# atonderski/future-object-detection

Measured on AMD Instinct MI355X. Metric: frame-sequences/sec fwd+bwd, T=6 900x1600, higher is better.
Workload: dtype bf16; 1 GPU; spatiotemporal ConditionalDETR (ResNet-50, 6 enc + 6 dec layers, 128 queries), T=6 frames 900x1600, batch 2/GPU, num_images K=5 (5 past frames live), random-init weights; step = forward (incl. Hungarian set loss, post-proc, AP bookkeeping) + backward + clip + AdamW; global_batch=2, frames=6, num_images=5, parallelism=dp1

## Files before the change

future-object-detection_amd/csrc/api.cpp:

```cpp
#include <stdarg.h>
#include <stdio.h>
#include <string.h>

#include "../../include/fod.h"

static thread_local char g_err[512] = "";

void fod_set_error(const char* fmt, ...) {
  va_list ap;
  va_start(ap, fmt);
  vsnprintf(g_err, sizeof(g_err), fmt, ap);
  va_end(ap);
}

extern "C" size_t fod_last_error(char* buf, size_t cap) {
  const size_t n = strlen(g_err);
  if (buf && cap) {
    const size_t c = n < cap - 1 ? n : cap - 1;
    memcpy(buf, g_err, c);
    buf[c] = 0;
  }
  return n;
}

extern "C" int fod_abi_version(void) { return FOD_ABI_VERSION; }

extern "C" size_t fod_workspace_bytes(int kind) {
  switch (kind) {
    case FOD_WS_NT_SPLIT: return (size_t)FOD_NT_SPLIT_WS_FLOATS * sizeof(float);
    case FOD_WS_NT_SPLIT_TICKETS: return (size_t)FOD_NT_SPLIT_TICKETS * sizeof(unsigned);
    case FOD_WS_TN_PARTIALS: return FOD_TN_WS_BYTES;
    case FOD_WS_ATTN_SPLIT_PER_TILE: return (size_t)FOD_ATTN_SPLIT_WS_FLOATS_PER_TILE * sizeof(float);
    default: return 0;
  }
}
```

future-object-detection_amd/csrc/gemm_tn_big.hip:

```cpp
#include <stdlib.h>

#include <type_traits>

#include "common.h"
#include "gemm_tn.h"
#include "lds_dma.h"

namespace {

using namespace fodtn;

constexpr int MS = 64;
constexpr int tn_stages(int bi, int bj) { return bi + bj == 512 ? 2 : 3; }
constexpr int tn_stage_bytes(int bi, int bj) { return MS * (bi + bj) * 2; }

template <int PITCH>
FOD_DEVINL Frag<__bf16> tr_frag(const unsigned char* tile, int a0, int ks) {
  typedef __attribute__((address_space(3))) short4_t* lds_s4;
  const short4_t lo = __builtin_amdgcn_ds_read_tr16_b64_v4i16((lds_s4)(tile + a0 + ks * 16 * PITCH));
  const short4_t hi = __builtin_amdgcn_ds_read_tr16_b64_v4i16((lds_s4)(tile + a0 + ks * 16 * PITCH + 4 * PITCH));
  typedef __attribute__((ext_vector_type(8))) short short8_t;
  const short8_t v = __builtin_shufflevector(lo, hi, 0, 1, 2, 3, 4, 5, 6, 7);
  Frag<__bf16> f;
  __builtin_memcpy(&f, &v, 16);
  return f;
}

template <int MODE, int BI, int BJ>
__global__ __launch_bounds__(512) void tn_big_kernel(const TnParams p) {
  static_assert((BI + BJ == 384 && (BI == 128 || BI == 256)) || (BI == 256 && BJ == 256),
                "tile shapes: 128 x 256, 256 x 128 or 256 x 256");
  constexpr int NSTAGE = tn_stages(BI, BJ), STAGE_BYTES = tn_stage_bytes(BI, BJ);
  constexpr int PG = BI * 2, PX = BJ * 2;
  constexpr int G_BYTES = MS * PG;
  constexpr int G_DMA = BI / 64, X_DMA = BJ / 64;
  constexpr int N_DMA = G_DMA + X_DMA;
  constexpr int WTJ = BI * BJ / 8 / 64;
  constexpr int NB = WTJ / 32;
  constexpr int WJ = BJ / WTJ;
  constexpr unsigned OOB = 0xFFFFFFF0u;
  extern __shared__ __attribute__((aligned(16))) unsigned char smem[];

  const int tid = threadIdx.x;
  const int lane = tid & 63;
  const int wave = __builtin_amdgcn_readfirstlane(tid >> 6);
  const int wi = wave / WJ, wj = wave % WJ;
  BLK_STAMP(0);
  const int ntile = p.ti * p.tj;
  const int per = (ntile * p.nsplit + 7) >> 3;
  const int item = p.xcd_order ? (int)(blockIdx.x & 7) * per + (int)(blockIdx.x >> 3) : (int)blockIdx.x;
  if (p.xcd_order && (int)(blockIdx.x >> 3) >= per) return;
  const int split = item / ntile;
  const int tile = item - split * ntile;
  const int bx = tile % p.tj, by = tile / p.tj;
  if (split >= p.nsplit) return;
  const int j0 = bx * BJ, i0 = by * BI;
  const int mb = split * p.m_per_split;
  const int mend = min(p.M, mb + p.m_per_split);
  const int nst = (mend - mb + MS - 1) / MS;

  const v4i rsG = make_rsrc(p.G, p.g_bytes), rsX = make_rsrc(p.X, p.x_bytes);
  const unsigned lds0 = (unsigned)(uintptr_t)(lds_ptr)smem;

  unsigned g_off[G_DMA];
  int g_m[G_DMA];
#pragma unroll
  for (int i = 0; i < G_DMA; ++i) {
    constexpr int CPR = PG / 16, RPP = 1024 / PG;
    const int row = (wave + 8 * i) * RPP + lane / CPR;
    const int sc = (lane % CPR) ^ ((row & 3) << 2);
    const int col = i0 + sc * 8;
    g_m[i] = col < p.N1 ? mb + row : (1 << 30);
    g_off[i] = (unsigned)(((long)(mb + row) * p.ldg + col) * 2);
  }
  const unsigned g_step = (unsigned)((long)MS * p.ldg * 2);

  unsigned x_off[X_DMA];
  int x_m[X_DMA];
// ... 209 lines not shown
      for (int a = 0; a < 2; ++a)
#pragma unroll
        for (int r = 0; r < 16; ++r)
          mine[(wi * 64 + a * 32 + acc_row(r, lane)) * BJ + wj * WTJ + b * 32 + (lane & 31)] = acc[a][b][r] * rs[a][r];
  } else {
#pragma unroll
    for (int b = 0; b < NB; ++b) {
      const int j = j0 + wj * WTJ + b * 32 + (lane & 31);
#pragma unroll
      for (int a = 0; a < 2; ++a)
#pragma unroll
        for (int r = 0; r < 16; ++r) {
          const int i = i0 + wi * 64 + a * 32 + acc_row(r, lane);
          if (i < p.N1 && j < p.K2) atomicAdd(p.dW + (long)i * p.ldw + j, acc[a][b][r] * rs[a][r]);
        }
    }
  }
#ifdef FOD_STAMPS
  asm volatile("s_waitcnt vmcnt(0)" ::: "memory");
  BLK_STAMP(3);
#endif
}

template <int BI, int BJ>
__global__ __launch_bounds__(256) void tn_reduce_kernel(const TnParams p) {
  __shared__ f32x4 red[3][64];
  const int c4 = p.K2 >> 2;
  const int chunks = (c4 + 63) >> 6;
  const int i = blockIdx.x / chunks;
  const int j4 = (blockIdx.x - i * chunks) * 64 + (threadIdx.x & 63);
  const int q = threadIdx.x >> 6;
  const bool in = j4 < c4;
  const int j = min(j4, c4 - 1) * 4;
  const int ntile = p.ti * p.tj;
  const int tile = (i / BI) * p.tj + j / BJ;
  const float* src = p.ws + (long)tile * (BI * BJ) + (i % BI) * BJ + j % BJ;
  const long stride = (long)ntile * (BI * BJ);
  f32x4 acc = {0.f, 0.f, 0.f, 0.f};
  int s = q;
  for (; s + 12 < p.nsplit; s += 16) {
    const f32x4 v0 = *reinterpret_cast<const f32x4*>(src + (s + 0) * stride);
    const f32x4 v1 = *reinterpret_cast<const f32x4*>(src + (s + 4) * stride);
    const f32x4 v2 = *reinterpret_cast<const f32x4*>(src + (s + 8) * stride);
    const f32x4 v3 = *reinterpret_cast<const f32x4*>(src + (s + 12) * stride);
    acc += v0;
    acc += v1;
    acc += v2;
    acc += v3;
  }
  for (; s < p.nsplit; s += 4) acc += *reinterpret_cast<const f32x4*>(src + s * stride);
  if (q > 0) red[q - 1][threadIdx.x & 63] = acc;
  __syncthreads();
  if (q > 0 || !in) return;
  acc += red[0][threadIdx.x];
  acc += red[1][threadIdx.x];
  acc += red[2][threadIdx.x];
  float* dst = p.dW + (long)i * p.ldw + j;
  if (p.accumulate) acc += *reinterpret_cast<const f32x4*>(dst);
  *reinterpret_cast<f32x4*>(dst) = acc;
}

template <int MODE, int BI, int BJ>
int launch_shape(const TnParams& p, hipStream_t stream) {
  static LdsLimitOnce lds_once;
  const size_t lds = (size_t)tn_stages(BI, BJ) * tn_stage_bytes(BI, BJ);
  if (int rc = fod_lds_limit_once(lds_once, reinterpret_cast<const void*>(&tn_big_kernel<MODE, BI, BJ>), lds, "gemm_tn_big")) return rc;
  const int ntile = p.ti * p.tj;
  const dim3 grid(p.xcd_order ? 8 * ceil_div((long)ntile * p.nsplit, 8) : ntile * p.nsplit);
  TnParams q = p;
  q.ws = nullptr;
  const char* env_ws = getenv("FOD_TN_WS");
  const size_t need = (size_t)ntile * p.nsplit * BI * BJ * sizeof(float);
  const bool aligned = ((uintptr_t)p.dW % 16) == 0 && p.ldw % 4 == 0;
  if (p.nsplit > 1 && p.ws_caller && need <= p.ws_caller_bytes && aligned && ((uintptr_t)p.ws_caller % 16) == 0 &&
      !(env_ws && env_ws[0] == '0'))
    q.ws = p.ws_caller;
  hipLaunchKernelGGL((tn_big_kernel<MODE, BI, BJ>), grid, dim3(512), lds, stream, q);
  FOD_LAUNCH_CHECK();
  if (q.ws) {
    hipLaunchKernelGGL((tn_reduce_kernel<BI, BJ>), dim3(p.N1 * ceil_div(p.K2 / 4, 64)), dim3(256), 0, stream, q);
    FOD_LAUNCH_CHECK();
  }
// ... 10 lines not shown
  const int sq = env_sq ? atoi(env_sq) : 0;
  const bool square = (sq == 2 && p.N1 >= 256 && p.K2 >= 256) ||
                      (sq == 1 && p.N1 % 256 == 0 && p.K2 % 256 == 0 && p.M >= 256 * 64);
  for (int shape = square ? 2 : 0; shape < (square ? 3 : 2); ++shape) {
    const int bi = shape == 0 ? 128 : 256, bj = shape == 2 ? 256 : 384 - bi;
    const int ti = ceil_div(p.N1, bi), tj = ceil_div(p.K2, bj);
    const int ntile = ti * tj;
    int s = 256 / ntile;
    const int max_s = p.M / 256;
    if (s > max_s) s = max_s;
    if (s < 1) s = 1;
    const int mps = ceil_div(ceil_div(p.M, s), MS) * MS;
    const int ns = ceil_div(p.M, mps);
    const int rounds = ceil_div((long)ntile * ns, 256);
    const double cost = rounds * (mps / MS * 0.55 + 17.0);
    if (cost < best_cost) {
      best_cost = cost;
      best = Plan{bi, bj, ti, tj, ns, mps};
    }
  }
  return best;
}

}

namespace fodtn {

bool big_applies(int mode, int dtype, const TnParams& p) {
  const char* env = getenv("FOD_TN_BIG");
  if (env && env[0] == '0') return false;
  if (dtype != FOD_BF16 || p.g_seg_cols) return false;
  if (p.N1 % 8 != 0 || p.K2 % 8 != 0 || p.ldg % 8 != 0) return false;
  if (mode == MODE_DENSE && p.ldx % 8 != 0) return false;
  if (mode == MODE_CONV && p.Cs % 8 != 0) return false;
  if (mode == MODE_CONV && (long)p.Hs * p.Ws * p.Cs * 2 >= (1L << 31)) return false;
  if (env && env[0] == '2') return p.M >= 1;
  const char* env_min = getenv("FOD_TN_BIG_MIN");
  return p.M >= 8192 && p.N1 >= 128 && p.K2 >= 128 && (double)p.M * p.N1 * p.K2 >= (env_min ? atof(env_min) : 2.0e9);
}

int launch_big_mode(int mode, const TnParams& p, hipStream_t stream) {
  TnParams q = p;
  const Plan pl = plan(p);
  q.ti = pl.ti; q.tj = pl.tj; q.nsplit = pl.nsplit; q.m_per_split = pl.m_per_split;
  const char* env_x = getenv("FOD_TN_XCD");
  q.xcd_order = (env_x && env_x[0] == '0') ? 0 : 1;
// ... 20 lines not shown
```

future-object-detection_amd/future_od/native/backbone.py:

```python
import os

import torch
import torch.nn as nn
from torch.autograd import Function

from . import functional as Fn
from . import ops

RESNET_SPECS = {"resnet18": ("basic", (2, 2, 2, 2), 1),
                "resnet34": ("basic", (3, 4, 6, 3), 1),
                "resnet50": ("bottleneck", (3, 4, 6, 3), 4)}
STAGE_WIDTH = (64, 128, 256, 512)


class FrozenBatchNorm2d(nn.Module):

    def __init__(self, n):
        super().__init__()
        self.register_buffer("weight", torch.ones(n))
        self.register_buffer("bias", torch.zeros(n))
        self.register_buffer("running_mean", torch.zeros(n))
        self.register_buffer("running_var", torch.ones(n))
        self.eps = 1e-5

# ... 80 lines not shown
            return ()
        c = getattr(self, "_pixel_norm", None)
        if c is None or c[0].device != video.device:
            c = (torch.tensor(self.PIXEL_MEAN, dtype=torch.float32, device=video.device),
                 torch.tensor(self.PIXEL_STD, dtype=torch.float32, device=video.device))
            object.__setattr__(self, "_pixel_norm", c)
        return c


FUSED_STEM_POOL = os.environ.get("FOD_FUSED_STEM_POOL", "1") != "0"

FRONT_FRAMES = int(os.environ.get("FOD_FRONT_FRAMES", "0")) or (1 << 30)


def _conv_fwd(x, cw, bn, dtype, relu, residual=None, cin_pad=None, out=None):
    scale, shift = bn.scale_shift()
    w = Fn.prep_conv(cw.weight, dtype, scale, False, cin_pad=cin_pad)
    geom = ops.conv_geom(x.shape, cw.weight.shape[0], cw.k, cw.stride, cw.pad)
    return ops.conv2d_fwd(x, w, geom, shift=shift, residual=residual, relu=relu, work_cin=cw.weight.shape[1],
                          out=out), geom


FUSED_BOTTLENECK = os.environ.get("FOD_FUSED_BOTTLENECK", "2")


def _fusable(blk, x, dtype, force=False):
    if (FUSED_BOTTLENECK == "0" and not force) or dtype != torch.bfloat16 or blk.kind == "basic":
        return False
    if FUSED_BOTTLENECK == "1" and not force and blk.downsample is None:
        return False
    main, ds = blk.convs()
    c1, c2, c3 = main[0][0], main[1][0], main[2][0]
    cin = x.shape[-1]
    if c1.weight.shape[0] != 64 or c3.weight.shape[0] != 256 or c2.stride != 1 or c1.stride != 1:
        return False
    if ds is None:
        return cin == 256
    return cin == 64 and ds[0].k == 1 and ds[0].stride == 1


def _fused_bottleneck(blk, x, dtype, out=None):
    main, ds = blk.convs()
    ws, bs = [], []
    for cw, bn in main + ([ds] if ds is not None else []):
        scale, shift = bn.scale_shift()
        ws.append(Fn.prep_conv(cw.weight, dtype, scale, False))
# ... 112 lines not shown
            x, acts, geoms, ds_geom = block_fwd(blk, x, pads=dom)
            if blk.convs()[0][0][0].weight.requires_grad:
                tape.append((blk, acts, geoms, ds_geom, dom))
        if dom is not None:
            x = _parity_merge(x, *dom)
        geom_p = ops.conv_geom(x.shape, proj.weight.shape[0], 1, 1, 0)
        wp = Fn.prep_conv(proj.weight, dtype, None, False)
        feat = ops.conv2d_fwd(x, wp, geom_p, shift=proj.bias.detach())
        ctx.body, ctx.proj, ctx.dtype = body, proj, dtype
        ctx.tape, ctx.x_last, ctx.geom_p = tape, x, geom_p
        ctx.train_weights = train_weights
        return feat

    @staticmethod
    def backward(ctx, dfeat):
        dtype, proj = ctx.dtype, ctx.proj
        dev = dfeat.device
        g = dfeat.contiguous()
        grads = {}
        sync = Fn.GRAD_SYNC
        if sync is not None:
            sync.flush(Fn.ARENA)

        def wgrad(gy, xin, cw, geom, scale):
            co, ci, kh, kw = cw.weight.shape
            dw = Fn.zeros_f32((co, kh, kw, ci), dev)
            ops.conv2d_wgrad_acc(gy, xin, dw, geom, row_scale=scale, zeroed=True)
            grads[id(cw.weight)] = dw.view(co, ci, 1, 1) if kh == 1 and kw == 1 else dw.permute(0, 3, 1, 2)

        if proj.weight.requires_grad:
            wgrad(g, ctx.x_last, proj, ctx.geom_p, None)
            db = Fn.zeros_f32((proj.weight.shape[0],), dev)
            ops.colsum_acc(g.view(-1, g.shape[-1]), db)
            grads[id(proj.bias)] = db
        tape = ctx.tape
        if tape:
            g = ops.conv2d_dgrad(g, Fn.prep_conv(proj.weight, dtype, None, True), ctx.geom_p, relu_mask=ctx.x_last)
        gdom = None
        for bi in range(len(tape) - 1, -1, -1):
            blk, acts, geoms, ds_geom, dom = tape[bi]
            if dom is not None and gdom is None:
                g, gdom = _parity_split(g), dom
            elif dom is None and gdom is not None:
                g, gdom = _parity_merge(g, *gdom), None
            main, ds = blk.convs()
            need_dx = bi > 0
            g_out = g
            gcur = g_out
            for j in range(len(main) - 1, -1, -1):
                cw, bn = main[j]
                scale, _ = bn.scale_shift()
                wgrad(gcur, acts[j], cw, geoms[j], scale)
                if j > 0:
                    gcur = ops.conv2d_dgrad(gcur, Fn.prep_conv(cw.weight, dtype, scale, True), geoms[j],
                                            relu_mask=acts[j])
            if ds is not None:
                wgrad(g_out, acts[0], ds[0], ds_geom, ds[1].scale_shift()[0])
            if need_dx:
                cw, bn = main[0]
                sc = bn.scale_shift()[0]
                w1t = Fn.prep_conv(cw.weight, dtype, sc, True)
                if ds is not None and ds[0].k == 1 and ds[0].stride == 2 and cw.stride == 1 and cw.k == 1:
                    g = ops.conv2d_dgrad(gcur, w1t, geoms[0], relu_mask=acts[0])
                    scd = ds[1].scale_shift()[0]
                    ops.conv2d_dgrad(g_out, Fn.prep_conv(ds[0].weight, dtype, scd, True), ds_geom, residual=g,
                                     relu_mask=acts[0], out=g)
                else:
                    if ds is not None:
                        scd = ds[1].scale_shift()[0]
                        d_idt = ops.conv2d_dgrad(g_out, Fn.prep_conv(ds[0].weight, dtype, scd, True), ds_geom)
                    else:
                        d_idt = g_out
                    g = ops.conv2d_dgrad(gcur, w1t, geoms[0], residual=d_idt, relu_mask=acts[0])
            if sync is not None:
                sync.maybe_flush(Fn.ARENA)
        ctx.tape = None
        out = [None, None, None, None]
        for w in ctx.train_weights:
            out.append(grads.get(id(w)))
        return tuple(out)


def backbone_trainable(body, proj):
    ws = []
    for _stage, blk in body.blocks():
        main, ds = blk.convs()
        for cw, _bn in main + ([ds] if ds is not None else []):
            if cw.weight.requires_grad:
                ws.append(cw.weight)
    ws += [proj.weight, proj.bias]
    return ws


def run_backbone(video, body, proj, dtype):
    feat = BackboneFn.apply(video, body, proj, dtype, *backbone_trainable(body, proj))
    if Fn.BACKBONE_CUT is not None and feat.requires_grad:
# ... 3 lines not shown
```

future-object-detection_amd/future_od/native/lib.py:

```python
import ctypes as C
import os

_HERE = os.path.dirname(os.path.abspath(__file__))
LIB_PATH = os.path.normpath(os.path.join(_HERE, "..", "..", "lib", "libfod_hip.so"))
ABI_VERSION = 4

F32, BF16 = 0, 1
EW_ADD, EW_MUL, EW_RELU_MASK, EW_SCALE, EW_ADD3, EW_RELU, EW_COPY_B = range(7)


class FodError(RuntimeError):
    pass


class Epilogue(C.Structure):
    _fields_ = [("scale", C.c_void_p), ("shift", C.c_void_p), ("residual", C.c_void_p),
                ("ld_residual", C.c_long), ("residual_row_mod", C.c_int), ("relu_mask", C.c_void_p),
                ("ld_mask", C.c_long), ("relu", C.c_int), ("out_f32", C.c_int),
                ("split_ws", C.c_void_p), ("split_tickets", C.c_void_p)]


class ConvGeom(C.Structure):
    _fields_ = [("Nimg", C.c_int), ("H", C.c_int), ("W", C.c_int), ("Cin", C.c_int),
                ("Ho", C.c_int), ("Wo", C.c_int), ("Cout", C.c_int),
                ("kh", C.c_int), ("kw", C.c_int), ("stride", C.c_int), ("pad", C.c_int)]


class AttnShape(C.Structure):
    _fields_ = [("B", C.c_int), ("H", C.c_int), ("Tq", C.c_int), ("S", C.c_int),
                ("q_batch_stride", C.c_long), ("q_token_stride", C.c_long),
                ("k_batch_stride", C.c_long), ("k_token_stride", C.c_long),
                ("v_batch_stride", C.c_long), ("v_token_stride", C.c_long),
                ("o_batch_stride", C.c_long), ("o_token_stride", C.c_long),
                ("scale", C.c_float),
                ("k2_batch_stride", C.c_long), ("k2_token_stride", C.c_long),
                ("dk2_batch_stride", C.c_long), ("dk2_token_stride", C.c_long),
                ("drop_p", C.c_float), ("drop_seed", C.c_ulonglong), ("drop_seed_dev", C.c_void_p),
                ("split_ws", C.c_void_p), ("split_tickets", C.c_void_p), ("dq_scale", C.c_float)]


class PermuteJob(C.Structure):
    _fields_ = [("src", C.c_void_p), ("dst", C.c_void_p), ("scale", C.c_void_p),
                ("src_dtype", C.c_int), ("dst_dtype", C.c_int),
                ("d0", C.c_int), ("d1", C.c_int), ("d2", C.c_int),
                ("valid1", C.c_int), ("valid2", C.c_int), ("scale_axis", C.c_int),
                ("s0", C.c_long), ("s1", C.c_long), ("s2", C.c_long),
                ("t0", C.c_long), ("t1", C.c_long)]

# ... 7 lines not shown


_i, _l, _f, _p = C.c_int, C.c_long, C.c_float, C.c_void_p
_EP, _CG, _AS = _p, _p, _p

SIGNATURES = {
    "fod_gemm_nt": [_i, _p, _l, _i, _p, _l, _p, _l, _i, _i, _i, _EP, _p],
    "fod_gemm_tn_acc": [_i, _p, _l, _p, _l, _p, _l, _i, _i, _i, _p, _p, _i, _p, C.c_size_t, _p],
    "fod_gemm_nt_grouped": [_i, _p, _l, _i, _l, _p, _l, _p, _l, _i, _l, _i, _i, _i, _EP, _i, _l, _p],
    "fod_gemm_nt_batched": [_i, _i, _p, _l, _l, _p, _l, _l, _p, _l, _l, _i, _i, _i, _EP, _l, _l, _l, _p],
    "fod_gemm_tn_grouped": [_i, _p, _l, _i, _l, _p, _l, _p, _l, _i, _i, _i, _p, _i, _p],
    "fod_gemm_tn_multi": [_p, _p, _p, _i, _p],
    "fod_gemm_tn_multi_long": [_p, _p, _p, _i, _p],
    "fod_tn_plan_long": [_i, _i, _p, _p],
    "fod_colsum_acc": [_i, _p, _l, _i, _i, _i, _p, _p],
    "fod_conv2d_fwd": [_i, _p, _p, _p, _CG, _EP, _p],
    "fod_conv2d_dgrad": [_i, _p, _p, _p, _CG, _EP, _p],
    "fod_conv_stem_fwd": [_i, _p, _p, _p, _i, _i, _i, _i, _i, _i, _EP, _p],
    "fod_stem_pool_fwd": [_i, _p, _p, _p, _p, _i, _i, _i, _i, _i, _i, _p],
    "fod_linear_add_norm_fwd": [_i, _p, _l, _p, _p, _p, _p, _p, _p, _p, _p, _p, _i, _i, _i, _f, _p, _p, _p, _p],
    "fod_linear_add_norm_bwd": [_i, _p, _p, _p, _p, _p, _p, _p, _p, _p, _p, _i, _i, _i, _p, _p, _p],
    "fod_clip_to_stem_layout": [_i, _i, _p, _p, _i, _i, _i, _i, _i, _i, _i, _l, _l, _p, _p, _p],
    "fod_conv2d_wgrad_acc": [_i, _p, _p, _p, _CG, _p, _i, _p, C.c_size_t, _p],
    "fod_bottleneck_fused_fwd": [_i, _p, _p, _p, _p, _p, _p, _p, _p, _p, _p, _i, _i, _i, _i, _i, _i, _p],
    "fod_maxpool3x3s2": [_i, _p, _p, _i, _i, _i, _i, _i, _i, _p],
    "fod_dropout": [_i, _p, _p, _l, C.c_ulonglong, _p, _f, _p],
    "fod_multi_permute3": [_p, _p, _p, _i, _p],
    "fod_multi_permute_chunk": [],
    "fod_multi_permute_tiles": [_i, _i, _i, _l, _l, _l],
    "fod_nchw_to_nhwc": [_i, _p, _p, _i, _i, _i, _i, _i, _i, _l, _l, _p],
    "fod_u8_nchw_to_nhwc": [_i, _p, _p, _i, _i, _i, _i, _i, _i, _l, _l, _p, _p, _p],
    "fod_permute3_cast": [_i, _i, _p, _p, _i, _i, _i, _l, _l, _l, _i, _p, _i, _p],
    "fod_attn_fwd": [_i, _p, _p, _p, _p, _p, _p, _p, _AS, _p],
    "fod_attn_bwd": [_i, _p, _p, _p, _p, _p, _p, _p, _p, _p, _p, _p, _p, _p, _p, _AS, _p],
    "fod_attn_bwd_dq": [_i, _p, _p, _p, _p, _p, _p, _p, _p, _p, _p, _p, _AS, _p],
    "fod_attn_bwd_dkv_multi": [_i, _i, _p, _AS, _p],
    "fod_attn_fp8_pack_bytes": [_AS, _i, _p, _p],
    "fod_attn_quant_fp8": [_p, _p, _p, _p, _p, _p, _p, _p, _p, _p, _p, _p, _AS, _p],
    "fod_attn_fwd_fp8": [_p, _p, _i, _p, _p, _AS, _p],
    "fod_colsum_groups_multi": [_i, _i, _p, _i, _i, _i, _p],
    "fod_mlp2_mul_fwd": [_i, _p, _p, _p, _p, _p, _p, _i, _p, _p, _p, _i, _i, _p],
    "fod_mlp2_mul_bwd": [_i, _p, _p, _i, _p, _p, _p, _p, _p, _p, _p, _p, _i, _i, _p],
    "fod_layernorm_fwd": [_i, _p, _p, _i, _i, _p, _p, _p, _p, _p, _p, _i, _i, _f, _i, _p],
    "fod_layernorm_bwd": [_i, _p, _p, _p, _p, _p, _p, _p, _p, _i, _i, _i, _p],
    "fod_eltwise": [_i, _i, _p, _p, _p, _p, _l, _i, _i, _i, _f, _p],
    "fod_posenc_table": [_i, _p, _i, _i, _i, _f, _p],
# ... 6 lines not shown
    "fod_lap_solve_batch_host": [_p, _i, _i, _i, _p, _p, _i],
    "fod_lap_solve_batch_dev": [_p, _i, _i, _i, _i, _p, _p, _p, _p],
    "fod_pack_targets": [_p, _p, _p, _i, _i, _f, _f, _p, _p, _p, _p, _p],
    "fod_host_flag_create": [_p],
    "fod_host_flag_destroy": [_p],
    "fod_host_alloc": [_p, C.c_size_t],
    "fod_host_free": [_p],
    "fod_copy_from_host_i32": [_p, _p, _i, _p],
    "fod_host_flag_set": [_p, C.c_uint32],
    "fod_stream_wait_flag": [_p, C.c_uint32, _p],
    "fod_stream_wait_supported": [_i],
    "fod_match_after_event": [_i, _p, _p, _i, _i, _i, _p, _p, _p, _p, C.c_uint32, _i],
    "fod_set_loss_fwd": [_p, _p, _p, _p, _p, _p, _p, _i, _i, _i, _i, _f, _p, _f, _p],
    "fod_set_loss_bwd": [_p, _p, _p, _p, _p, _p, _p, _p, _i, _i, _i, _i, _f, _p, _f, _p],
    "fod_od_map": [_p, _p, _p, _p, _p, _p, _p, _p, _p, _i, _i, _i, _i, _i, _f, _f, _p],
    "fod_post_proc": [_p, _p, _p, _p, _i, _i, _f, _f, _p],
    "fod_tracker_cost": [_p, _p, _p, _p, _p, _i, _i, _i, _i, _p],
    "fod_tracker_extrapolate": [_p, _p, _p, _p, _p, _p, _p, _p, _i, _i, _i, _i, _i, _p],
    "fod_multi_sqnorm_acc": [_p, _p, _p, _p, _i, _p, _p],
    "fod_multi_sqnorm_det": [_p, _p, _p, _p, _i, _p, _p, _p],
    "fod_multi_adamw": [_p, _p, _p, _p, _p, _i, _f, _f, _f, _f, _f, _p, _p, _f, _p],
}
EXPORTS = sorted(list(SIGNATURES) + ["fod_last_error", "fod_abi_version", "fod_multi_chunk", "fod_workspace_bytes"])
WS_NT_SPLIT, WS_NT_SPLIT_TICKETS, WS_TN_PARTIALS, WS_ATTN_SPLIT_PER_TILE = range(4)


def _load():
    if not os.path.isfile(LIB_PATH):
        raise FodError(
            f"{LIB_PATH} not found: build it with `python -c 'import __graft_entry__ as g; g.build()'` "
            "(or future-object-detection_amd/build.sh). There is no fallback path.")
    import torch
    lib = C.CDLL(LIB_PATH)
    lib.fod_abi_version.restype = C.c_int
    lib.fod_abi_version.argtypes = []
    if lib.fod_abi_version() != ABI_VERSION:
        raise FodError(f"libfod_hip.so ABI {lib.fod_abi_version()} != binding ABI {ABI_VERSION}: rebuild")
    lib.fod_last_error.restype = C.c_size_t
    lib.fod_last_error.argtypes = [C.c_char_p, C.c_size_t]
    lib.fod_workspace_bytes.restype = C.c_size_t
    lib.fod_workspace_bytes.argtypes = [C.c_int]
    for name, args in SIGNATURES.items():
        fn = getattr(lib, name)
        fn.restype = C.c_int
        fn.argtypes = args
    return lib

# ... 76 lines not shown
```

future-object-detection_amd/future_od/native/ops.py:

```python
import ctypes as C
import math

import torch

from . import lib as L
from .lib import F32, BF16, AttnShape, ConvGeom, Epilogue


def call(name, *args, **kw):
    return L.call(name, *args, **kw)

_DT = {torch.float32: F32, torch.bfloat16: BF16}


def dt(t):
    try:
        return _DT[t.dtype]
    except KeyError:
        raise L.FodError(f"unsupported activation dtype {t.dtype}") from None


_raw_stream = getattr(torch._C, "_cuda_getCurrentRawStream", None)


# ... 24 lines not shown
        raise L.FodError(f"{name}: expected a contiguous tensor, got strides {t.stride()} for {tuple(t.shape)}")
    if dtype is not None and t.dtype != dtype:
        raise L.FodError(f"{name}: expected {dtype}, got {t.dtype}")
    return t


_WS = {}


def _workspace(kind, device, captured=None):
    if captured is None:
        captured = torch.cuda.is_current_stream_capturing()
    key = (kind, device.index, "graph" if captured else stream())
    hit = _WS.get(key)
    if hit is None:
        nbytes = L.LIB.fod_workspace_bytes(kind)
        hit = torch.zeros(nbytes // 4, dtype=torch.int32, device=device)
        _WS[key] = hit
    return hit


def preallocate_graph_workspaces(device):
    device = torch.device(device)
    for kind in (L.WS_NT_SPLIT, L.WS_NT_SPLIT_TICKETS, L.WS_TN_PARTIALS):
        _workspace(kind, device, captured=True)


def _epi(scale=None, shift=None, residual=None, ld_residual=0, residual_row_mod=0, relu_mask=None,
         ld_mask=0, relu=False, out_f32=False, split_for=None):
    want_split = (split_for is not None and split_for[3] >= 1024
                  and ((split_for[1] + 63) // 64) * ((split_for[2] + 63) // 64) <= 64)
    if (scale is None and shift is None and residual is None and relu_mask is None and not relu and not out_f32
            and not want_split):
        return None
    ws = tk = None
    if want_split:
        ws, tk = _workspace(L.WS_NT_SPLIT, split_for[0]), _workspace(L.WS_NT_SPLIT_TICKETS, split_for[0])
    e = Epilogue(ptr(scale), ptr(shift), ptr(residual), ld_residual, residual_row_mod,
                 ptr(relu_mask), ld_mask, int(relu), int(out_f32), ptr(ws), ptr(tk))
    return _Addr(e)


def tn_workspace(device):
    ws = _workspace(L.WS_TN_PARTIALS, device)
    return ws.data_ptr(), ws.numel() * 4


# ... 217 lines not shown
    dx = out if out is not None else torch.empty((geom.Nimg, geom.H, geom.W, geom.Cin), dtype=dy.dtype, device=dy.device)
    for v in (residual, relu_mask):
        if v is not None:
            _chk(v, "residual/mask", dy.dtype); assert v.shape == dx.shape
    call("fod_conv2d_dgrad", dt(dy), ptr(dy), ptr(w_t), ptr(dx), _Addr(geom),
         _epi(None, None, residual, geom.Cin, 0, relu_mask, geom.Cin, False), stream(), work=_conv_flops(geom))
    return dx


def conv2d_wgrad_acc(dy, x, dw, geom, row_scale=None, zeroed=False):
    _chk(dy, "dy"); _chk(x, "x", dy.dtype); _chk(dw, "dw", torch.float32)
    assert tuple(dy.shape) == (geom.Nimg, geom.Ho, geom.Wo, geom.Cout)
    assert tuple(x.shape) == (geom.Nimg, geom.H, geom.W, geom.Cin)
    assert dw.numel() == geom.Cout * geom.kh * geom.kw * geom.Cin
    if row_scale is not None:
        _chk(row_scale, "row_scale", torch.float32); assert row_scale.numel() == geom.Cout
    ws, ws_bytes = tn_workspace(dy.device) if dy.numel() // geom.Cout >= 8192 else (None, 0)
    call("fod_conv2d_wgrad_acc", dt(dy), ptr(dy), ptr(x), ptr(dw), _Addr(geom), ptr(row_scale),
         0 if zeroed else 1, ws, ws_bytes, stream(),
         work=_conv_flops(geom))
    return dw


def bottleneck_fused_fwd(x, w1, b1, w2, b2, w3, b3, wd=None, bd=None, out=None):
    _chk(x, "x", torch.bfloat16)
    n, h, w, cin = x.shape
    for t, name, numel in ((w1, "w1", 64 * cin), (w2, "w2", 64 * 9 * 64), (w3, "w3", 256 * 64)):
        _chk(t, name, torch.bfloat16); assert t.numel() == numel, (name, t.shape)
    for t, name, numel in ((b1, "b1", 64), (b2, "b2", 64), (b3, "b3", 256)):
        _chk(t, name, torch.float32); assert t.numel() == numel
    if wd is not None:
        _chk(wd, "wd", torch.bfloat16); _chk(bd, "bd", torch.float32)
        assert wd.numel() == 256 * cin and bd.numel() == 256
    if out is None:
        out = torch.empty((n, h, w, 256), dtype=x.dtype, device=x.device)
    else:
        _chk(out, "out", x.dtype); assert tuple(out.shape) == (n, h, w, 256)
    flops = 2.0 * n * h * w * (cin * 64 + 9 * 64 * 64 + 64 * 256 + (cin * 256 if wd is not None else 0))
    call("fod_bottleneck_fused_fwd", dt(x), ptr(x), ptr(w1), ptr(b1), ptr(w2), ptr(b2), ptr(w3), ptr(b3), ptr(wd),
         ptr(bd), ptr(out), n, h, w, cin, 64, 256, stream(), work=flops, tag="fod_conv2d_fwd")
    return out


def maxpool3x3s2(x):
    _chk(x, "x")
    n, h, w, c = x.shape
# ... 575 lines not shown
```

include/fod.h:

```cpp
#ifndef FOD_H_
#define FOD_H_

#include <stddef.h>
#include <stdint.h>

#ifdef __cplusplus
extern "C" {
#endif

typedef struct ihipStream_t* fod_stream_t;

enum { FOD_F32 = 0, FOD_BF16 = 1 };
enum { FOD_OK = 0, FOD_ERR_ARG = 1, FOD_ERR_LAUNCH = 2, FOD_ERR_RUNTIME = 3 };

size_t fod_last_error(char* buf, size_t cap);
int fod_abi_version(void);
#define FOD_ABI_VERSION 4

typedef struct fod_epilogue {
  const float* scale;
  const float* shift;
  const void* residual;
  long ld_residual;
  int residual_row_mod;
  const void* relu_mask;
  long ld_mask;
  int relu;
  int out_f32;
  void* split_ws;
  void* split_tickets;
} fod_epilogue;
#define FOD_NT_SPLIT_WS_FLOATS (64 * 8 * 4096)
#define FOD_NT_SPLIT_TICKETS 64
#define FOD_TN_WS_BYTES ((size_t)64 << 20)
enum { FOD_WS_NT_SPLIT = 0, FOD_WS_NT_SPLIT_TICKETS = 1, FOD_WS_TN_PARTIALS = 2, FOD_WS_ATTN_SPLIT_PER_TILE = 3 };
size_t fod_workspace_bytes(int kind);

int fod_gemm_nt(int dtype, const void* A, long lda, int a_row_mod, const void* B, long ldb, void* C,
                long ldc, int M, int N, int K, const fod_epilogue* epi, fod_stream_t stream);

int fod_gemm_tn_acc(int dtype, const void* G, long ldg, const void* X, long ldx, float* dW, long ldw,
                    int M, int N1, int K2, const float* row_scale, float* colsum, int accumulate,
                    void* ws ,
                    size_t ws_bytes, fod_stream_t stream);

int fod_gemm_nt_grouped(int dtype, const void* A, long lda, int a_seg_len, long a_seg_stride, const void* B,
                        long ldb, void* C, long ldc, int c_seg_cols, long c_seg_stride, int M, int N, int K,
                        const fod_epilogue* epi,
                        int res_nseg, long res_seg_stride, fod_stream_t stream);
int fod_gemm_nt_batched(int dtype, int batches, const void* A, long lda, long a_batch, const void* B, long ldb,
                        long b_batch, void* C, long ldc, long c_batch, int M, int N, int K, const fod_epilogue* epi,
                        long shift_batch, long residual_batch, long mask_batch, fod_stream_t stream);
int fod_gemm_tn_grouped(int dtype, const void* G, long ldg, int g_seg_cols, long g_seg_stride, const void* X,
                        long ldx, float* dW, long ldw, int M, int N1, int K2, float* colsum, int accumulate,
                        fod_stream_t stream);

typedef struct fod_tn_job {
  const void* G;
// ... 28 lines not shown
} fod_permute_job;
int fod_multi_permute3(const fod_permute_job* jobs, const int* blk_job, const int* blk_chunk, int nblocks,
                       fod_stream_t stream);
int fod_multi_permute_chunk(void);
int fod_multi_permute_tiles(int d0, int d1, int d2, long s0, long s1, long s2);

typedef struct fod_conv_geom {
  int Nimg, H, W, Cin;
  int Ho, Wo, Cout;
  int kh, kw, stride, pad;
} fod_conv_geom;

int fod_conv2d_fwd(int dtype, const void* x, const void* w, void* y, const fod_conv_geom* g,
                   const fod_epilogue* epi, fod_stream_t stream);
int fod_conv_stem_fwd(int dtype, const void* xp, const void* w, void* y, int Nimg, int Hp, int Wp, int Ho, int Wo,
                      int Cout, const fod_epilogue* epi, fod_stream_t stream);
int fod_stem_pool_fwd(int dtype, const void* xp, const void* w, const float* shift, void* y, int Nimg, int Hp, int Wp,
                      int Ho, int Wo, int Cout, fod_stream_t stream);
int fod_conv2d_dgrad(int dtype, const void* dy, const void* w_t, void* dx, const fod_conv_geom* g,
                     const fod_epilogue* epi, fod_stream_t stream);
int fod_conv2d_wgrad_acc(int dtype, const void* dy, const void* x, float* dw, const fod_conv_geom* g,
                         const float* row_scale, int accumulate, void* ws ,
                         size_t ws_bytes, fod_stream_t stream);

int fod_bottleneck_fused_fwd(int dtype, const void* x, const void* w1, const float* b1, const void* w2,
                             const float* b2, const void* w3, const float* b3, const void* wd, const float* bd,
                             void* out, int Nimg, int H, int W, int Cin, int mid, int Cout, fod_stream_t stream);

int fod_maxpool3x3s2(int dtype, const void* x, void* y, int Nimg, int H, int W, int C, int Ho, int Wo,
                     fod_stream_t stream);

int fod_nchw_to_nhwc(int dtype, const float* src, void* dst, int F, int C, int H, int W, int Cp, int inner,
                     long stride_outer, long stride_inner, fod_stream_t stream);

int fod_u8_nchw_to_nhwc(int dtype, const unsigned char* src, void* dst, int F, int C, int H, int W, int Cp,
                        int inner, long stride_outer, long stride_inner, const float* mean, const float* std,
                        fod_stream_t stream);

int fod_clip_to_stem_layout(int dtype, int src_u8, const void* src, void* dst, int F, int C, int H, int W, int Hp,
                            int Wp, int inner, long stride_outer, long stride_inner, const float* mean,
                            const float* std, fod_stream_t stream);

int fod_permute3_cast(int src_dtype, int dst_dtype, const void* src, void* dst, int d0, int d1, int d2,
                      long s0, long s1, long s2, int valid2, const float* scale, int scale_axis,
                      fod_stream_t stream);

// ... 152 lines not shown
```

Measured before the change: 109.2 frame-sequences/s.

## Batch backbone conv weight-gradient GEMMs into one grouped split-K launch

Adds a grouped conv wgrad entry point that packs up to 44 per-layer weight-gradient jobs into a single persistent-style TN GEMM launch, followed by a single grouped reduction. A host-side planner chooses split-K factors by simulating the makespan across 8 XCDs and 32 CUs each. The backbone backward pass collects all small-enough wgrads and issues them together at the end instead of one launch per conv. The goal is to cut launch overhead and fill the GPU better on small wgrads, at the cost of a 128 MB workspace, a linear job search in every block, and extra host planning work per call.

Result: no change. 110.0 frame-sequences/s, median of 5 (+0.8%).

```diff
diff --git a/future-object-detection_amd/csrc/api.cpp b/future-object-detection_amd/csrc/api.cpp
--- a/future-object-detection_amd/csrc/api.cpp
+++ b/future-object-detection_amd/csrc/api.cpp
@@ -30,6 +30,7 @@
     case FOD_WS_NT_SPLIT: return (size_t)FOD_NT_SPLIT_WS_FLOATS * sizeof(float);
     case FOD_WS_NT_SPLIT_TICKETS: return (size_t)FOD_NT_SPLIT_TICKETS * sizeof(unsigned);
     case FOD_WS_TN_PARTIALS: return FOD_TN_WS_BYTES;
+    case FOD_WS_TN_MULTI: return FOD_TN_MULTI_WS_BYTES;
     case FOD_WS_ATTN_SPLIT_PER_TILE: return (size_t)FOD_ATTN_SPLIT_WS_FLOATS_PER_TILE * sizeof(float);
     default: return 0;
   }
diff --git a/future-object-detection_amd/csrc/gemm_tn_big.hip b/future-object-detection_amd/csrc/gemm_tn_big.hip
--- a/future-object-detection_amd/csrc/gemm_tn_big.hip
+++ b/future-object-detection_amd/csrc/gemm_tn_big.hip
@@ -1,6 +1,8 @@
 #include <stdlib.h>
 
+#include <algorithm>
 #include <type_traits>
+#include <vector>
 
 #include "common.h"
 #include "gemm_tn.h"
@@ -27,7 +29,7 @@
 }
 
 template <int MODE, int BI, int BJ>
-__global__ __launch_bounds__(512) void tn_big_kernel(const TnParams p) {
+FOD_DEVINL void tn_big_body(const TnParams& p, const int split, const int tile) {
   static_assert((BI + BJ == 384 && (BI == 128 || BI == 256)) || (BI == 256 && BJ == 256),
                 "tile shapes: 128 x 256, 256 x 128 or 256 x 256");
   constexpr int NSTAGE = tn_stages(BI, BJ), STAGE_BYTES = tn_stage_bytes(BI, BJ);
@@ -47,13 +49,7 @@
   const int wi = wave / WJ, wj = wave % WJ;
   BLK_STAMP(0);
   const int ntile = p.ti * p.tj;
-  const int per = (ntile * p.nsplit + 7) >> 3;
-  const int item = p.xcd_order ? (int)(blockIdx.x & 7) * per + (int)(blockIdx.x >> 3) : (int)blockIdx.x;
-  if (p.xcd_order && (int)(blockIdx.x >> 3) >= per) return;
-  const int split = item / ntile;
-  const int tile = item - split * ntile;
   const int bx = tile % p.tj, by = tile / p.tj;
-  if (split >= p.nsplit) return;
   const int j0 = bx * BJ, i0 = by * BI;
   const int mb = split * p.m_per_split;
   const int mend = min(p.M, mb + p.m_per_split);
@@ -309,13 +305,24 @@
 #endif
 }
 
+template <int MODE, int BI, int BJ>
+__global__ __launch_bounds__(512) void tn_big_kernel(const TnParams p) {
+  const int ntile = p.ti * p.tj;
+  const int per = (ntile * p.nsplit + 7) >> 3;
+  const int item = p.xcd_order ? (int)(blockIdx.x & 7) * per + (int)(blockIdx.x >> 3) : (int)blockIdx.x;
+  if (p.xcd_order && (int)(blockIdx.x >> 3) >= per) return;
+  const int split = item / ntile;
+  if (split >= p.nsplit) return;
+  tn_big_body<MODE, BI, BJ>(p, split, item - split * ntile);
+}
+
 template <int BI, int BJ>
-__global__ __launch_bounds__(256) void tn_reduce_kernel(const TnParams p) {
+FOD_DEVINL void tn_reduce_body(const TnParams& p, const int blk) {
   __shared__ f32x4 red[3][64];
   const int c4 = p.K2 >> 2;
   const int chunks = (c4 + 63) >> 6;
-  const int i = blockIdx.x / chunks;
-  const int j4 = (blockIdx.x - i * chunks) * 64 + (threadIdx.x & 63);
+  const int i = blk / chunks;
+  const int j4 = (blk - i * chunks) * 64 + (threadIdx.x & 63);
   const int q = threadIdx.x >> 6;
   const bool in = j4 < c4;
   const int j = min(j4, c4 - 1) * 4;
@@ -345,6 +352,98 @@
   float* dst = p.dW + (long)i * p.ldw + j;
   if (p.accumulate) acc += *reinterpret_cast<const f32x4*>(dst);
   *reinterpret_cast<f32x4*>(dst) = acc;
+}
+
+template <int BI, int BJ>
+__global__ __launch_bounds__(256) void tn_reduce_kernel(const TnParams p) {
+  tn_reduce_body<BI, BJ>(p, blockIdx.x);
+}
+
+struct WgJob {
+  const void* G;
+  const void* X;
+  float* dW;
+  const float* rscale;
+  int M, blk0, m_per_split, nsplit;
+  unsigned short Hs, Ws, Hd, Wd, Cs, N1;
+  unsigned char kh, kw, stride, pad;
+};
+static_assert(sizeof(WgJob) == 64, "job layout");
+constexpr int WG_MAX_JOBS = 44;
+constexpr int WG_BI = 128, WG_BJ = 256;
+struct WgJobs {
+  WgJob j[WG_MAX_JOBS];
+  float* ws;
+  int njobs, nblk;
+};
+
+FOD_DEVINL TnParams wg_params(const WgJob& j, float* ws) {
+  TnParams p{};
+  p.G = j.G; p.X = j.X; p.dW = j.dW; p.rscale = j.rscale;
+  p.M = j.M; p.N1 = j.N1; p.K2 = j.kh * j.kw * j.Cs;
+  p.ldg = j.N1; p.ldw = p.K2;
+  p.Hs = j.Hs; p.Ws = j.Ws; p.Cs = j.Cs; p.Hd = j.Hd; p.Wd = j.Wd;
+  p.kh = j.kh; p.kw = j.kw; p.stride = j.stride; p.pad = j.pad;
+  p.g_bytes = (unsigned)((long)j.M * j.N1 * 2);
+  p.x_bytes = (unsigned)((long)(j.M / (j.Hd * j.Wd)) * j.Hs * j.Ws * j.Cs * 2);
+  p.ti = (j.N1 + WG_BI - 1) / WG_BI;
+  p.tj = (p.K2 + WG_BJ - 1) / WG_BJ;
+  p.nsplit = j.nsplit; p.m_per_split = j.m_per_split;
+  p.ws = ws + (long)j.blk0 * (WG_BI * WG_BJ);
+  return p;
+}
+
+__global__ __launch_bounds__(512) void tn_big_kernel_grouped(const WgJobs t) {
+  const int b = blockIdx.x;
+  int jb = 0;
+  while (jb + 1 < t.njobs && b >= t.j[jb + 1].blk0) ++jb;
+  const TnParams p = wg_params(t.j[jb], t.ws);
+  const int ntile = p.ti * p.tj;
+  const int lb = b - t.j[jb].blk0;
+  const int per = (ntile * p.nsplit + 7) >> 3;
+  const int item = (lb & 7) * per + (lb >> 3);
+  const int split = item / ntile;
+  if ((lb >> 3) >= per || split >= p.nsplit) return;
+  tn_big_body<MODE_CONV, WG_BI, WG_BJ>(p, split, item - split * ntile);
+}
+
+constexpr int WG_RED_F4 = 1024;
+__global__ __launch_bounds__(256) void tn_reduce_kernel_grouped(const WgJobs t) {
+  int b = blockIdx.x, jb = 0;
+  for (; jb + 1 < t.njobs; ++jb) {
+    const WgJob& j = t.j[jb];
+    const int n = (j.N1 * (j.kh * j.kw * j.Cs / 4) + WG_RED_F4 - 1) / WG_RED_F4;
+    if (b < n) break;
+    b -= n;
+  }
+  const TnParams p = wg_params(t.j[jb], t.ws);
+  const int c4 = p.K2 >> 2, total = p.N1 * c4;
+  const long stride = (long)p.ti * p.tj * (WG_BI * WG_BJ);
+  const float* src[4];
+  bool in[4];
+  f32x4 acc[4];
+#pragma unroll
+  for (int u = 0; u < 4; ++u) {
+    const int e = b * WG_RED_F4 + u * 256 + (int)threadIdx.x;
+    in[u] = e < total;
+    const int ee = in[u] ? e : 0;
+    const int i = ee / c4, j = (ee - i * c4) * 4;
+    src[u] = p.ws + (long)((i / WG_BI) * p.tj + j / WG_BJ) * (WG_BI * WG_BJ) + (i % WG_BI) * WG_BJ + j % WG_BJ;
+    acc[u] = f32x4{0.f, 0.f, 0.f, 0.f};
+  }
+  for (int s = 0; s < p.nsplit; ++s) {
+    f32x4 v[4];
+#pragma unroll
+    for (int u = 0; u < 4; ++u) v[u] = *reinterpret_cast<const f32x4*>(src[u] + s * stride);
+#pragma unroll
+    for (int u = 0; u < 4; ++u) acc[u] += v[u];
+  }
+#pragma unroll
+  for (int u = 0; u < 4; ++u) {
+    if (!in[u]) continue;
+    const int e = b * WG_RED_F4 + u * 256 + (int)threadIdx.x;
+    *reinterpret_cast<f32x4*>(p.dW + (long)e * 4) = acc[u];
+  }
 }
 
 template <int MODE, int BI, int BJ>
@@ -401,6 +500,150 @@
   return best;
 }
 
+constexpr int WG_ITEM_OVERHEAD = 7;
+
+struct WgPlan {
+  std::vector<int> order, mps, ns;
+  int nblk = 0;
+};
+
+static int wg_tiles(const fod_wgrad_job& j) {
+  return ceil_div(j.g.Cout, WG_BI) * ceil_div(j.g.kh * j.g.kw * j.g.Cin, WG_BJ);
+}
+
+static bool wg_try(const std::vector<fod_wgrad_job>& jobs, int r, long cap_slots, WgPlan& pl, double& makespan) {
+  const int n = (int)jobs.size();
+  pl.mps.assign(n, 0);
+  pl.ns.assign(n, 0);
+  for (int i = 0; i < n; ++i) {
+    const int M = jobs[i].g.Nimg * jobs[i].g.Ho * jobs[i].g.Wo;
+    const int st = ceil_div(M, MS);
+    int s = ceil_div(st, r);
+    if (s < 1) s = 1;
+    pl.mps[i] = ceil_div(ceil_div(M, s), MS) * MS;
+    pl.ns[i] = ceil_div(M, pl.mps[i]);
+  }
+  pl.order.resize(n);
+  for (int i = 0; i < n; ++i) pl.order[i] = i;
+  std::stable_sort(pl.order.begin(), pl.order.end(), [&](int a, int b) { return pl.mps[a] > pl.mps[b]; });
+  long slots = 0;
+  for (int i : pl.order) slots += 8L * ceil_div((long)wg_tiles(jobs[i]) * pl.ns[i], 8);
+  if (slots > cap_slots || slots > (1L << 30)) return false;
+  pl.nblk = (int)slots;
+  makespan = 0;
+  for (int x = 0; x < 8; ++x) {
+    double cu[32] = {0};
+    for (int i : pl.order) {
+      const int M = jobs[i].g.Nimg * jobs[i].g.Ho * jobs[i].g.Wo;
+      const int ntile = wg_tiles(jobs[i]);
+      const int items = ntile * pl.ns[i], per = ceil_div(items, 8);
+      for (int it = x * per; it < std::min(items, (x + 1) * per); ++it) {
+        const int split = it / ntile;
+        const int rows = std::min(pl.mps[i], M - split * pl.mps[i]);
+        int k = 0;
+        for (int c = 1; c < 32; ++c)
+          if (cu[c] < cu[k]) k = c;
+        cu[k] += ceil_div(rows, MS) + WG_ITEM_OVERHEAD;
+      }
+    }
+    for (int c = 0; c < 32; ++c) makespan = std::max(makespan, cu[c]);
+  }
+  return true;
+}
+
+static bool wg_plan(const std::vector<fod_wgrad_job>& jobs, long cap_slots, WgPlan& best) {
+  int max_st = 1;
+  for (const auto& j : jobs) max_st = std::max(max_st, ceil_div(j.g.Nimg * j.g.Ho * j.g.Wo, MS));
+  std::vector<std::pair<int, double>> ok;
+  WgPlan pl;
+  for (double rr = 8.0;; rr *= 1.03) {
+    const int r = std::min((int)rr, max_st);
+    double ms;
+    if (wg_try(jobs, r, cap_slots, pl, ms)) ok.push_back({r, ms});
+    if (r >= max_st) break;
+  }
+  if (ok.empty()) return false;
+  double best_ms = 1e300;
+  for (const auto& o : ok) best_ms = std::min(best_ms, o.second);
+  int best_r = -1;
+  double ms;
+  for (const auto& o : ok)
+    if (o.second <= 1.02 * best_ms) best_r = o.first;
+  return wg_try(jobs, best_r, cap_slots, best, ms);
+}
+
+}
+
+extern "C" int fod_conv2d_wgrad_multi(int dtype, int njobs, const fod_wgrad_job* jobs, void* ws, size_t ws_bytes,
+                                      hipStream_t stream) {
+  FOD_REQUIRE(dtype == FOD_BF16, "conv_wgrad_multi: bf16 only (dtype %d)", dtype);
+  FOD_REQUIRE(njobs > 0 && jobs, "conv_wgrad_multi: no jobs");
+  FOD_REQUIRE(ws && ((uintptr_t)ws % 16) == 0, "conv_wgrad_multi: a 16-byte aligned workspace is required");
+  const long tile_bytes = (long)WG_BI * WG_BJ * sizeof(float);
+  const long cap = (long)(ws_bytes / tile_bytes);
+  for (int i = 0; i < njobs; ++i) {
+    const fod_wgrad_job& j = jobs[i];
+    const fod_conv_geom& g = j.g;
+    FOD_REQUIRE(j.dy && j.x && j.dw, "conv_wgrad_multi: null operand in job %d", i);
+    FOD_REQUIRE(((uintptr_t)j.dy % 16) == 0 && ((uintptr_t)j.x % 16) == 0 && ((uintptr_t)j.dw % 16) == 0,
+                "conv_wgrad_multi: operands of job %d must be 16-byte aligned", i);
+    FOD_REQUIRE(g.Cin % 8 == 0 && g.Cout % 8 == 0, "conv_wgrad_multi: job %d channels %d/%d must be multiples of 8", i,
+                g.Cin, g.Cout);
+    FOD_REQUIRE(g.Ho == (g.H + 2 * g.pad - g.kh) / g.stride + 1 && g.Wo == (g.W + 2 * g.pad - g.kw) / g.stride + 1,
+                "conv_wgrad_multi: geometry mismatch in job %d", i);
+    FOD_REQUIRE(g.H < 65536 && g.W < 65536 && g.Ho < 65536 && g.Wo < 65536 && g.Cin < 65536 && g.Cout < 65536 &&
+                    g.kh < 256 && g.kw < 256 && g.stride < 256 && g.pad < 256 && g.Nimg > 0 && g.stride > 0,
+                "conv_wgrad_multi: job %d extents out of range", i);
+    const long M = (long)g.Nimg * g.Ho * g.Wo;
+    FOD_REQUIRE(M < (1L << 31), "conv_wgrad_multi: pixel count of job %d overflows int", i);
+    FOD_REQUIRE(M * g.Cout * 2 < 0xFFFFFFF0L - 16 && (long)g.Nimg * g.H * g.W * g.Cin * 2 < 0xFFFFFFF0L - 16 &&
+                    (long)g.H * g.W * g.Cin * 2 < (1L << 31),
+                "conv_wgrad_multi: operand of job %d larger than the 32-bit walks allow", i);
+  }
+  for (int c0 = 0; c0 < njobs;) {
+    std::vector<fod_wgrad_job> chunk;
+    long slots = 0;
+    for (int i = c0; i < njobs && (int)chunk.size() < WG_MAX_JOBS; ++i) {
+      const long s = 8L * ceil_div((long)wg_tiles(jobs[i]), 8);
+      if (slots + s > cap) break;
+      chunk.push_back(jobs[i]);
+      slots += s;
+    }
+    FOD_REQUIRE(!chunk.empty(), "conv_wgrad_multi: workspace of %zu bytes too small for job %d", ws_bytes, c0);
+    WgPlan pl;
+    FOD_REQUIRE(wg_plan(chunk, cap, pl), "conv_wgrad_multi: no plan");
+    WgJobs t{};
+    t.ws = reinterpret_cast<float*>(ws);
+    t.njobs = (int)chunk.size();
+    int blk = 0, red = 0;
+    for (int k = 0; k < t.njobs; ++k) {
+      const int i = pl.order[k];
+      const fod_wgrad_job& s = chunk[i];
+      WgJob& j = t.j[k];
+      j.G = s.dy; j.X = s.x; j.dW = s.dw; j.rscale = s.row_scale;
+      j.M = s.g.Nimg * s.g.Ho * s.g.Wo;
+      j.blk0 = blk;
+      j.m_per_split = pl.mps[i];
+      j.nsplit = pl.ns[i];
+      j.Hs = (unsigned short)s.g.H; j.Ws = (unsigned short)s.g.W; j.Hd = (unsigned short)s.g.Ho;
+      j.Wd = (unsigned short)s.g.Wo; j.Cs = (unsigned short)s.g.Cin; j.N1 = (unsigned short)s.g.Cout;
+      j.kh = (unsigned char)s.g.kh; j.kw = (unsigned char)s.g.kw;
+      j.stride = (unsigned char)s.g.stride; j.pad = (unsigned char)s.g.pad;
+      blk += 8 * ceil_div(wg_tiles(s) * pl.ns[i], 8);
+      red += ceil_div(s.g.Cout * (s.g.kh * s.g.kw * s.g.Cin / 4), WG_RED_F4);
+    }
+    t.nblk = blk;
+    static LdsLimitOnce lds_once;
+    const size_t lds = (size_t)tn_stages(WG_BI, WG_BJ) * tn_stage_bytes(WG_BI, WG_BJ);
+    if (int rc = fod_lds_limit_once(lds_once, reinterpret_cast<const void*>(&tn_big_kernel_grouped), lds, "conv_wgrad_multi"))
+      return rc;
+    hipLaunchKernelGGL(tn_big_kernel_grouped, dim3(blk), dim3(512), lds, stream, t);
+    FOD_LAUNCH_CHECK();
+    hipLaunchKernelGGL(tn_reduce_kernel_grouped, dim3(red), dim3(256), 0, stream, t);
+    FOD_LAUNCH_CHECK();
+    c0 += t.njobs;
+  }
+  return FOD_OK;
 }
 
 namespace fodtn {
diff --git a/future-object-detection_amd/future_od/native/backbone.py b/future-object-detection_amd/future_od/native/backbone.py
--- a/future-object-detection_amd/future_od/native/backbone.py
+++ b/future-object-detection_amd/future_od/native/backbone.py
@@ -126,6 +126,8 @@
 
 
 FUSED_BOTTLENECK = os.environ.get("FOD_FUSED_BOTTLENECK", "2")
+WGRAD_MULTI = os.environ.get("FOD_CONV_WGRAD_MULTI", "1") != "0"
+WGRAD_MULTI_ROWS = int(os.environ.get("FOD_CONV_WGRAD_MULTI_ROWS", "100000"))
 
 
 def _fusable(blk, x, dtype, force=False):
@@ -284,10 +286,16 @@
         if sync is not None:
             sync.flush(Fn.ARENA)
 
+        group = []
+        grouped = WGRAD_MULTI and dtype == torch.bfloat16
+
         def wgrad(gy, xin, cw, geom, scale):
             co, ci, kh, kw = cw.weight.shape
             dw = Fn.zeros_f32((co, kh, kw, ci), dev)
-            ops.conv2d_wgrad_acc(gy, xin, dw, geom, row_scale=scale, zeroed=True)
+            if grouped and geom.Nimg * geom.Ho * geom.Wo <= WGRAD_MULTI_ROWS:
+                group.append((gy, xin, dw, geom, scale))
+            else:
+                ops.conv2d_wgrad_acc(gy, xin, dw, geom, row_scale=scale, zeroed=True)
             grads[id(cw.weight)] = dw.view(co, ci, 1, 1) if kh == 1 and kw == 1 else dw.permute(0, 3, 1, 2)
 
         if proj.weight.requires_grad:
@@ -334,6 +342,11 @@
                     else:
                         d_idt = g_out
                     g = ops.conv2d_dgrad(gcur, w1t, geoms[0], residual=d_idt, relu_mask=acts[0])
+            if sync is not None and not group:
+                sync.maybe_flush(Fn.ARENA)
+        if group:
+            ops.conv2d_wgrad_multi(group)
+            group.clear()
             if sync is not None:
                 sync.maybe_flush(Fn.ARENA)
         ctx.tape = None
diff --git a/future-object-detection_amd/future_od/native/lib.py b/future-object-detection_amd/future_od/native/lib.py
--- a/future-object-detection_amd/future_od/native/lib.py
+++ b/future-object-detection_amd/future_od/native/lib.py
@@ -3,7 +3,7 @@
 
 _HERE = os.path.dirname(os.path.abspath(__file__))
 LIB_PATH = os.path.normpath(os.path.join(_HERE, "..", "..", "lib", "libfod_hip.so"))
-ABI_VERSION = 4
+ABI_VERSION = 5
 
 F32, BF16 = 0, 1
 EW_ADD, EW_MUL, EW_RELU_MASK, EW_SCALE, EW_ADD3, EW_RELU, EW_COPY_B = range(7)
@@ -24,6 +24,11 @@
     _fields_ = [("Nimg", C.c_int), ("H", C.c_int), ("W", C.c_int), ("Cin", C.c_int),
                 ("Ho", C.c_int), ("Wo", C.c_int), ("Cout", C.c_int),
                 ("kh", C.c_int), ("kw", C.c_int), ("stride", C.c_int), ("pad", C.c_int)]
+
+
+class WgradJob(C.Structure):
+    _fields_ = [("dy", C.c_void_p), ("x", C.c_void_p), ("dw", C.c_void_p), ("row_scale", C.c_void_p),
+                ("g", ConvGeom)]
 
 
 class AttnShape(C.Structure):
@@ -77,6 +82,7 @@
     "fod_linear_add_norm_bwd": [_i, _p, _p, _p, _p, _p, _p, _p, _p, _p, _p, _i, _i, _i, _p, _p, _p],
     "fod_clip_to_stem_layout": [_i, _i, _p, _p, _i, _i, _i, _i, _i, _i, _i, _l, _l, _p, _p, _p],
     "fod_conv2d_wgrad_acc": [_i, _p, _p, _p, _CG, _p, _i, _p, C.c_size_t, _p],
+    "fod_conv2d_wgrad_multi": [_i, _i, _p, _p, C.c_size_t, _p],
     "fod_bottleneck_fused_fwd": [_i, _p, _p, _p, _p, _p, _p, _p, _p, _p, _p, _i, _i, _i, _i, _i, _i, _p],
     "fod_maxpool3x3s2": [_i, _p, _p, _i, _i, _i, _i, _i, _i, _p],
     "fod_dropout": [_i, _p, _p, _l, C.c_ulonglong, _p, _f, _p],
@@ -129,7 +135,7 @@
     "fod_multi_adamw": [_p, _p, _p, _p, _p, _i, _f, _f, _f, _f, _f, _p, _p, _f, _p],
 }
 EXPORTS = sorted(list(SIGNATURES) + ["fod_last_error", "fod_abi_version", "fod_multi_chunk", "fod_workspace_bytes"])
-WS_NT_SPLIT, WS_NT_SPLIT_TICKETS, WS_TN_PARTIALS, WS_ATTN_SPLIT_PER_TILE = range(4)
+WS_NT_SPLIT, WS_NT_SPLIT_TICKETS, WS_TN_PARTIALS, WS_ATTN_SPLIT_PER_TILE, WS_TN_MULTI = range(5)
 
 
 def _load():
diff --git a/future-object-detection_amd/future_od/native/ops.py b/future-object-detection_amd/future_od/native/ops.py
--- a/future-object-detection_amd/future_od/native/ops.py
+++ b/future-object-detection_amd/future_od/native/ops.py
@@ -70,7 +70,7 @@
 
 def preallocate_graph_workspaces(device):
     device = torch.device(device)
-    for kind in (L.WS_NT_SPLIT, L.WS_NT_SPLIT_TICKETS, L.WS_TN_PARTIALS):
+    for kind in (L.WS_NT_SPLIT, L.WS_NT_SPLIT_TICKETS, L.WS_TN_PARTIALS, L.WS_TN_MULTI):
         _workspace(kind, device, captured=True)
 
 
@@ -334,6 +334,23 @@
     return dw
 
 
+def conv2d_wgrad_multi(jobs):
+    arr = (L.WgradJob * len(jobs))()
+    work = 0.0
+    for k, (dy, x, dw, geom, row_scale) in enumerate(jobs):
+        _chk(dy, "dy", torch.bfloat16); _chk(x, "x", torch.bfloat16); _chk(dw, "dw", torch.float32)
+        assert tuple(dy.shape) == (geom.Nimg, geom.Ho, geom.Wo, geom.Cout)
+        assert tuple(x.shape) == (geom.Nimg, geom.H, geom.W, geom.Cin)
+        assert dw.numel() == geom.Cout * geom.kh * geom.kw * geom.Cin
+        if row_scale is not None:
+            _chk(row_scale, "row_scale", torch.float32); assert row_scale.numel() == geom.Cout
+        arr[k] = L.WgradJob(ptr(dy), ptr(x), ptr(dw), ptr(row_scale), geom)
+        work += _conv_flops(geom)
+    ws = _workspace(L.WS_TN_MULTI, jobs[0][0].device)
+    call("fod_conv2d_wgrad_multi", BF16, len(jobs), C.addressof(arr), ws.data_ptr(), ws.numel() * 4, stream(),
+         work=work, tag="fod_conv2d_wgrad_acc")
+
+
 def bottleneck_fused_fwd(x, w1, b1, w2, b2, w3, b3, wd=None, bd=None, out=None):
     _chk(x, "x", torch.bfloat16)
     n, h, w, cin = x.shape
diff --git a/include/fod.h b/include/fod.h
--- a/include/fod.h
+++ b/include/fod.h
@@ -15,7 +15,7 @@
 
 size_t fod_last_error(char* buf, size_t cap);
 int fod_abi_version(void);
-#define FOD_ABI_VERSION 4
+#define FOD_ABI_VERSION 5
 
 typedef struct fod_epilogue {
   const float* scale;
@@ -33,7 +33,9 @@
 #define FOD_NT_SPLIT_WS_FLOATS (64 * 8 * 4096)
 #define FOD_NT_SPLIT_TICKETS 64
 #define FOD_TN_WS_BYTES ((size_t)64 << 20)
-enum { FOD_WS_NT_SPLIT = 0, FOD_WS_NT_SPLIT_TICKETS = 1, FOD_WS_TN_PARTIALS = 2, FOD_WS_ATTN_SPLIT_PER_TILE = 3 };
+#define FOD_TN_MULTI_WS_BYTES ((size_t)128 << 20)
+enum { FOD_WS_NT_SPLIT = 0, FOD_WS_NT_SPLIT_TICKETS = 1, FOD_WS_TN_PARTIALS = 2, FOD_WS_ATTN_SPLIT_PER_TILE = 3,
+       FOD_WS_TN_MULTI = 4 };
 size_t fod_workspace_bytes(int kind);
 
 int fod_gemm_nt(int dtype, const void* A, long lda, int a_row_mod, const void* B, long ldb, void* C,
@@ -108,6 +110,15 @@
 int fod_conv2d_wgrad_acc(int dtype, const void* dy, const void* x, float* dw, const fod_conv_geom* g,
                          const float* row_scale, int accumulate, void* ws ,
                          size_t ws_bytes, fod_stream_t stream);
+typedef struct fod_wgrad_job {
+  const void* dy;
+  const void* x;
+  float* dw;
+  const float* row_scale;
+  fod_conv_geom g;
+} fod_wgrad_job;
+int fod_conv2d_wgrad_multi(int dtype, int njobs, const fod_wgrad_job* jobs, void* ws, size_t ws_bytes,
+                           fod_stream_t stream);
 
 int fod_bottleneck_fused_fwd(int dtype, const void* x, const void* w1, const float* b1, const void* w2,
                              const float* b2, const void* w3, const float* b3, const void* wd, const float* bd,
```
